# aliabdelkader/FusionTransformer

Hardware: AMD Instinct MI355X
Metric: frames/sec fwd+bwd (SemanticKITTI synth), whole job (higher is better)
Workload: dtype f32

## Files before the change

### fusiontransformer_amd/_lib.py

```python
from __future__ import annotations

import ctypes as C
import os

import torch

_HERE = os.path.dirname(os.path.abspath(__file__))
LIB_PATH = os.path.join(_HERE, "csrc", "libftx.so")

_i32, _i64, _f32, _vp, _sz = C.c_int32, C.c_int64, C.c_float, C.c_void_p, C.c_size_t

SIGNATURES = {
    "ftx_version": (C.c_int, []),
    "ftx_last_error": (C.c_char_p, []),
    "ftx_stream_scratch_bytes": (_sz, []),
    "ftx_stream_scratch_attach": (C.c_int, [_vp, _vp, _sz]),
    "ftx_stream_scratch_reset": (C.c_int, [_vp]),
    "ftx_stream_scratch_release": (C.c_int, [_vp]),
    "ftx_hash": (C.c_int, [_vp, _i64, _vp, _vp]),
    "ftx_hash_kernel": (C.c_int, [_vp, _i64, _vp, _i32, _vp, _vp]),
    "ftx_floor_coords": (C.c_int, [_vp, _i64, _i32, _vp, _vp]),
    "ftx_hashtable_capacity": (_i64, [_i64]),
    "ftx_hashtable_build": (C.c_int, [_vp, _i64, _vp, _vp, _i64, _vp]),
    "ftx_hashtable_query": (C.c_int, [_vp, _i64, _vp, _vp, _i64, _vp, _vp]),
# ... 18 lines not shown
    "ftx_devoxelize_fwd": (C.c_int, [_vp, _vp, _vp, _i64, _i32, _i64, _vp, _vp]),
    "ftx_devoxelize_bwd": (C.c_int, [_vp, _vp, _vp, _i64, _i32, _i64, _vp, _vp]),
    "ftx_segment_workspace_bytes": (_sz, [_i64, _i64]),
    "ftx_segment_build": (C.c_int, [_vp, _i64, _i64, _vp, _vp, _vp, _sz, _vp]),
    "ftx_voxelize_fwd_sorted": (C.c_int, [_vp, _vp, _vp, _i64, _i32, _i64, _vp, _vp]),
    "ftx_devoxelize_bwd_sorted": (C.c_int, [_vp, _vp, _vp, _vp, _i64, _i32, _i64, _vp, _vp]),
    "ftx_segment_sum": (C.c_int, [_vp, _vp, _vp, _i64, _i32, _i64, _vp, _vp]),
    "ftx_lift_cells": (C.c_int, [_vp, _vp, _i64, _i32, _i32, _i32, _i32, _i32, _vp, _vp]),
    "ftx_lift_gather_fwd": (C.c_int, [_vp, _vp, _vp, _i64, _i32, _i32, _i32, _i32, _i32, _i32, _vp, _vp]),
    "ftx_lift_gather_bwd": (C.c_int, [_vp, _vp, _vp, _i64, _i32, _i32, _i32, _i32, _i32, _i32, _vp, _vp]),
    "ftx_resample_nearest_fwd": (C.c_int, [_vp, _i32, _i32, _i32, _i32, _i32, _i32, _vp, _vp]),
    "ftx_resample_nearest_bwd": (C.c_int, [_vp, _i32, _i32, _i32, _i32, _i32, _i32, _vp, _vp]),
    "ftx_sample_down_workspace_bytes": (_sz, []),
    "ftx_sample_down_fwd": (C.c_int, [_vp, _i32, _i32, _i32, _i32, _i32, _vp, _vp, _vp, _vp, _vp, _vp, _f32, _f32, _i32, _vp, _vp, _vp, _sz, _vp]),
    "ftx_sample_down_bwd": (C.c_int, [_vp, _vp, _i32, _i32, _i32, _i32, _i32, _vp, _vp, _vp, _vp, _vp, _vp, _vp, _vp, _vp, _sz, _vp]),
    "ftx_affine_sample_fwd": (C.c_int, [_vp, _vp, _i32, _i32, _i32, _i32, _vp, _i32, _i32, _vp, _vp]),
    "ftx_affine_theta_workspace_bytes": (_sz, [_i32]),
    "ftx_affine_sample_bwd_theta": (C.c_int, [_vp, _vp, _i32, _i32, _i32, _i32, _vp, _vp, _i32, _i32, _vp, _vp, _sz, _vp]),
    "ftx_affine_lift_fwd": (C.c_int, [_vp, _vp, _i32, _i32, _i32, _i32, _vp, _vp, _vp, _i64, _i32, _i32, _vp, _vp]),
    "ftx_affine_lift_cells": (C.c_int, [_vp, _vp, _vp, _i64, _i32, _i32, _i32, _i32, _i32, _vp, _vp]),
    "ftx_affine_lift_bwd": (C.c_int, [_vp, _vp, _i32, _i32, _i32, _i32, _vp, _vp, _vp, _vp, _i64, _i32, _i32, _vp, _vp, _vp, _vp, _vp, _sz, _vp]),
    "ftx_loc_conv_pool_relu_fwd_workspace_bytes": (_sz, [_i32, _i32, _i32, _i32]),
    "ftx_loc_conv_pool_relu_fwd": (C.c_int, [_vp, _vp, _i32, _i32, _i32, _i32, _vp, _vp, _i32, _i32, _vp, _vp, _vp, _vp, _sz, _vp]),
    "ftx_loc_conv_pool_relu_bwd_weight_workspace_bytes": (_sz, [_i32, _i32, _i32, _i32, _i32, _i32]),
    "ftx_loc_conv_pool_relu_bwd_weight": (C.c_int, [_vp, _vp, _i32, _i32, _i32, _i32, _vp, _vp, _vp, _i32, _i32, _vp, _vp, _vp, _sz, _vp]),
    "ftx_loc_conv_pool_relu_bwd_data": (C.c_int, [_vp, _vp, _vp, _vp, _i32, _i32, _i32, _i32, _i32, _i32, _vp, _vp, _vp]),
    "ftx_spconv_pairs_gemm": (C.c_int, [_vp, _i64, _vp, _vp, _i32, _vp, _i64, _i32, _i32, _i32, _vp, _vp]),
    "ftx_spconv_pairs_gemm_scatter": (C.c_int, [_vp, _i64, _vp, _vp, _vp, _i32, _vp, _i64, _i32, _i32, _i32, _vp, _i64, _vp]),
    "ftx_spconv_ostat_supported": (_i32, [_i32, _i32, _i32, _i32]),
    "ftx_spconv_ostat_blocks": (_i32, [_i64]),
    "ftx_spconv_ostat": (C.c_int, [_vp, _i64, _vp, _i64, _vp, _i32, _i32, _i32, _i32, _i32, _vp, _vp, _i32, _vp]),
    "ftx_rows_gemm": (C.c_int, [_vp, _i64, _vp, _i32, _vp, _i32, _i32, _vp, _vp]),
    "ftx_spconv_gemm_block_cols": (_i32, [_i32, _i64, _i32]),
    "ftx_spconv_reduce": (C.c_int, [_vp, _vp, _i64, _i32, _i32, _vp, _vp]),
    "ftx_spconv_reduce_bn_eval": (C.c_int, [_vp, _vp, _i64, _i32, _i32, _vp, _vp, _vp, _vp, _vp, _f32, _i32, _vp, _vp]),
    "ftx_spconv_reduce_stats_blocks": (_i32, [_i64, _i32]),
    "ftx_spconv_reduce_stats": (C.c_int, [_vp, _vp, _i64, _i32, _i32, _vp, _vp, _i32, _vp]),
    "ftx_bn_train_fwd_totals": (C.c_int, [_vp, _vp, _vp, _vp, _vp, _vp, _f32, _f32, _i64, _i32, _i32, _vp, _vp, _vp, _vp, _vp]),
    "ftx_spconv_pairs_wgrad_workspace_bytes": (_sz, [_i64, _i32, _i32, _i32]),
    "ftx_spconv_pairs_wgrad": (C.c_int, [_vp, _i64, _vp, _vp, _i64, _vp, _vp, _i64, _i32, _i32, _i32, _vp, _vp, _sz, _vp]),
    "ftx_spconv_wgrad_resident_blocks": (_i32, [_i32, _i32]),
    "ftx_spconv_wgrad_table_blocks": (_i32, [_i32, _i32, _i32, _i32]),
    "ftx_spconv_pairs_gemm_bf16": (C.c_int, [_vp, _i64, _vp, _vp, _i32, _vp, _i64, _i32, _i32, _i32, _vp, _vp]),
    "ftx_spconv_pairs_gemm_scatter_bf16": (C.c_int, [_vp, _i64, _vp, _vp, _vp, _i32, _vp, _i64, _i32, _i32, _i32, _vp, _i64, _vp]),
    "ftx_rows_gemm_bf16": (C.c_int, [_vp, _i64, _vp, _i32, _vp, _i32, _i32, _vp, _vp]),
    "ftx_spconv_pairs_wgrad_bf16_workspace_bytes": (_sz, [_i64, _i32, _i32, _i32]),
    "ftx_spconv_pairs_wgrad_bf16": (C.c_int, [_vp, _i64, _vp, _vp, _i64, _vp, _vp, _i64, _i32, _i32, _i32, _vp, _vp, _sz, _vp]),
    "ftx_spconv_gemm_bf16_block_cols": (_i32, [_i32, _i64, _i32]),
    "ftx_spconv_wgrad_bf16_table_blocks": (_i32, [_i32, _i32, _i32, _i32]),
    "ftx_bn_workspace_bytes": (_sz, [_i64, _i32]),
    "ftx_bn_train_fwd": (C.c_int, [_vp, _vp, _vp, _vp, _vp, _vp, _f32, _f32, _i64, _i32, _i32, _vp, _vp, _vp, _vp, _sz, _vp]),
    "ftx_bn_eval_fwd": (C.c_int, [_vp, _vp, _vp, _vp, _vp, _vp, _f32, _i64, _i32, _i32, _vp, _vp]),
    "ftx_adam_chunk_elements": (_i32, []),
    "ftx_adam_tensor_bytes": (_i32, []),
    "ftx_adam_step": (C.c_int, [_vp, _vp, _vp, _i32, C.c_double, C.c_double, _f32, _f32, _vp]),
    "ftx_add_layernorm_fwd": (C.c_int, [_vp, _vp, _vp, _vp, _vp, _f32, _i64, _i32, _vp, _vp, _vp, _vp, _vp]),
    "ftx_layernorm_bwd_workspace_bytes": (_sz, [_i64, _i32]),
    "ftx_add_layernorm_bwd": (C.c_int, [_vp, _vp, _vp, _vp, _vp, _vp, _i64, _i32, _i32, _vp, _vp, _vp, _sz, _vp]),
    "ftx_colsum_workspace_bytes": (_sz, [_i64, _i32]),
    "ftx_colsum": (C.c_int, [_vp, _i64, _i32, _vp, _vp, _sz, _vp]),
    "ftx_attn_fwd": (C.c_int, [_vp, _i32, _i32, _i32, _i32, _f32, _vp, _vp, _vp]),
    "ftx_attn_bwd_workspace_bytes": (_sz, [_i32, _i32, _i32]),
    "ftx_attn_bwd": (C.c_int, [_vp, _vp, _vp, _vp, _i32, _i32, _i32, _i32, _f32, _vp, _vp, _sz, _vp]),
    "ftx_attn_fwd_tiled": (C.c_int, [_vp, _i32, _i32, _i32, _i32, _f32, _vp, _vp, _i32, _i32, _vp]),
    "ftx_attn_bwd_tiled": (C.c_int, [_vp, _vp, _vp, _vp, _i32, _i32, _i32, _i32, _f32, _vp, _vp, _sz, _i32, _i32, _vp]),
    "ftx_attn_fwd_bf16": (C.c_int, [_vp, _i32, _i32, _i32, _i32, _f32, _vp, _vp, _i32, _i32, _vp]),
# ... 105 lines not shown
```

### fusiontransformer_amd/csrc/ftx_spconv.hip

```cpp
#include <cstring>
#include <cstdlib>
#include "ftx_bn_eval_op.h"
#include "ftx_spconv_common.h"
#include <rocprim/device/device_scan.hpp>
#include <rocprim/iterator/transform_iterator.hpp>

using namespace ftx;

struct IsValid {
  __host__ __device__ int32_t operator()(int32_t v) const { return v >= 0 ? 1 : 0; }
};

extern "C" size_t ftx_kernel_map_count_workspace_bytes(int64_t n_out, int32_t k) {
  if (n_out <= 0 || k <= 0) return 256;
  size_t bytes = 0;
  const int32_t *in = nullptr;
  int32_t *out = nullptr;
  auto it = rocprim::make_transform_iterator(in, IsValid());
  if (rocprim::exclusive_scan(nullptr, bytes, it, out, 0, (size_t)(n_out * k), rocprim::plus<int32_t>()) != hipSuccess) return 0;
  return bytes + 256;
}

__global__ void koff_kernel(const int32_t *__restrict__ nbr, const int32_t *__restrict__ scan, int64_t n_out, int k, int32_t *__restrict__ koff) {
  int t = blockIdx.x * blockDim.x + threadIdx.x;
// ... 162 lines not shown
        int nn = e >> 3, k4 = (e & 7) * 4;
        *(float4 *)&Bs[nn * BS_STRIDE + k4] = rb[q];
      }
    }
  };

  load_chunk(0);
  for (int c0 = 0; c0 < ca; c0 += kPairBK) {
    store_chunk();
    __syncthreads();
    if (c0 + kPairBK < ca) load_chunk(c0 + kPairBK);
    const float *arow_p = &As[(wave * 32 + l31) * AS_STRIDE + 4 * half];
    const float *brow_p = &Bs[l31 * BS_STRIDE + 4 * half];
    float af[2][4], bf[2][NT][4];
    auto load_frag = [&](int buf, int t) {
      float4 a = *(const float4 *)(arow_p + 8 * t);
      af[buf][0] = a.x; af[buf][1] = a.y; af[buf][2] = a.z; af[buf][3] = a.w;
#pragma unroll
      for (int j = 0; j < NT; ++j) {
        float4 b = *(const float4 *)(brow_p + j * 32 * BS_STRIDE + 8 * t);
        bf[buf][j][0] = b.x; bf[buf][j][1] = b.y; bf[buf][j][2] = b.z; bf[buf][j][3] = b.w;
      }
    };
    load_frag(0, 0);
#pragma unroll
    for (int t = 0; t < kPairBK / 8; ++t) {
      if (t + 1 < kPairBK / 8) load_frag((t + 1) & 1, t + 1);
#pragma unroll
      for (int s = 0; s < 4; ++s)
#pragma unroll
        for (int j = 0; j < NT; ++j) acc[j] = __builtin_amdgcn_mfma_f32_32x32x2f32(bf[t & 1][j][s], af[t & 1][s], acc[j], 0, 0, 0);
    }
    __syncthreads();
  }
  pair_gemm_epilogue<NT>(acc, p0, cnt, n0, gather, rows_a, scatter, rows_out, bias, co, tmp);
}

#include "ftx_lastblock.h"


template <int KVOL>
__device__ __forceinline__ float4 reduce_row(const float *__restrict__ tmp, const int32_t *__restrict__ pos, int64_t n, int co, int kvol,
                                             int64_t r, int j) {
  float4 acc = make_float4(0.f, 0.f, 0.f, 0.f);
  if (KVOL > 0) {
    int32_t p[KVOL > 0 ? KVOL : 1];
#pragma unroll
    for (int k = 0; k < KVOL; ++k) p[k] = pos[(int64_t)k * n + r];
#pragma unroll
    for (int k = 0; k < KVOL; ++k) {
      if (p[k] >= 0) {
        float4 v = *(const float4 *)&tmp[(int64_t)p[k] * co + j];
        acc.x += v.x; acc.y += v.y; acc.z += v.z; acc.w += v.w;
      }
    }
  } else {
    for (int k = 0; k < kvol; ++k) {
      int32_t q = pos[(int64_t)k * n + r];
      if (q >= 0) {
        float4 v = *(const float4 *)&tmp[(int64_t)q * co + j];
        acc.x += v.x; acc.y += v.y; acc.z += v.z; acc.w += v.w;
      }
    }
  }
  return acc;
}
// ... 275 lines not shown
    float *dst = single ? dW + (int64_t)k * mat : part + (int64_t)blockIdx.x * mat;
    const int ab = m0 + wm * 32 * MI + MI * l31, gb = n0 + wn * 32 * NI;
#pragma unroll
    for (int i = 0; i < MI; ++i) {
      const int row = ab + i;
      if (row < ca) {
#pragma unroll
        for (int q = 0; q < 4; ++q) {
          float v[4 * NI];
#pragma unroll
          for (int e = 0; e < 4; ++e)
#pragma unroll
            for (int j = 0; j < NI; ++j) v[e * NI + j] = acc[i][j][4 * q + e];
          const int col = gb + NI * (8 * q + 4 * half);
#pragma unroll
          for (int t = 0; t < NI; ++t)
            if (col + 4 * t < cg) *(float4 *)&dst[(int64_t)row * cg + col + 4 * t] = make_float4(v[4 * t], v[4 * t + 1], v[4 * t + 2], v[4 * t + 3]);
        }
      }
    }
  }
}

struct SpconvF32 {
  static constexpr const char *pairs_name = "ftx_spconv_pairs_gemm", *scatter_name = "ftx_spconv_pairs_gemm_scatter", *rows_name = "ftx_rows_gemm",
                              *wgrad_name = "ftx_spconv_pairs_wgrad";
  static constexpr int wgrad_blocks[4][4] = {{8, 4, 3, 3}, {5, 3, 2, 2}, {4, 2, 1, 2}, {3, 2, 2, 2}};
  static constexpr int wgrad_step = 2 * WG_BR;
  template <int NT>
  static void gemm(dim3 grid, hipStream_t st, const PairsGemmArgs &a) {
    pairs_gemm_kernel<NT><<<grid, 256, 0, st>>>(a.A, a.rows_a, a.gather, a.W, a.w_transposed, a.koff, a.ca, a.co, a.kvol, a.out, a.bias, a.n_dense,
                                                a.scatter, a.rows_out);
  }
  template <int MI, int NI, int WMG, int WNG>
  static void wgrad(dim3 grid, hipStream_t st, const PairsWgradArgs &a) {
    pairs_wgrad_kernel<MI, NI, WMG, WNG><<<grid, 256, 0, st>>>(a.A, a.rows_a, a.idx_a, a.G, a.rows_g, a.idx_g, a.koff, a.ca, a.cg, a.kvol, a.tile_len,
                                                               a.part, a.dW, a.n_dense);
  }
};

extern "C" int32_t ftx_spconv_gemm_block_cols(int32_t co, int64_t n_pairs, int32_t kvol) { return spconv_gemm_block_cols(co, n_pairs, kvol); }

extern "C" int ftx_spconv_pairs_gemm(const float *A, int64_t rows_a, const int32_t *gather, const float *W, int32_t w_transposed,
                                     const int32_t *koff, int64_t n_pairs, int32_t ca, int32_t co, int32_t kvol, float *tmp, void *stream) {
  return spconv_pairs_entry<SpconvF32>(false, A, rows_a, gather, nullptr, W, w_transposed, koff, n_pairs, ca, co, kvol, tmp, 0, stream);
}

extern "C" int ftx_spconv_pairs_gemm_scatter(const float *A, int64_t rows_a, const int32_t *gather, const int32_t *scatter, const float *W,
                                             int32_t w_transposed, const int32_t *koff, int64_t n_pairs, int32_t ca, int32_t co, int32_t kvol,
                                             float *out, int64_t rows_out, void *stream) {
  return spconv_pairs_entry<SpconvF32>(true, A, rows_a, gather, scatter, W, w_transposed, koff, n_pairs, ca, co, kvol, out, rows_out, stream);
}

extern "C" int ftx_rows_gemm(const float *A, int64_t n, const float *W, int32_t w_transposed, const float *bias, int32_t ca, int32_t co,
                             float *out, void *stream) {
  return spconv_rows_entry<SpconvF32>(A, n, W, w_transposed, bias, ca, co, out, stream);
}

extern "C" int32_t ftx_spconv_wgrad_table_blocks(int32_t mi, int32_t wmg, int32_t ni, int32_t wng) {
  return spconv_wgrad_table_blocks<SpconvF32>(mi, wmg, ni, wng);
}
extern "C" int32_t ftx_spconv_wgrad_resident_blocks(int32_t ca, int32_t cg) { return spconv_wgrad_occ<SpconvF32>(spconv_wgrad_config(ca, cg)); }

extern "C" size_t ftx_spconv_pairs_wgrad_workspace_bytes(int64_t n_pairs, int32_t ca, int32_t cg, int32_t kvol) {
  return spconv_wgrad_workspace_bytes<SpconvF32>(n_pairs, ca, cg, kvol);
}

extern "C" int ftx_spconv_pairs_wgrad(const float *A, int64_t rows_a, const int32_t *idx_a, const float *G, int64_t rows_g, const int32_t *idx_g,
                                      const int32_t *koff, int64_t n_pairs, int32_t ca, int32_t cg, int32_t kvol, float *dW, void *workspace,
                                      size_t workspace_bytes, void *stream) {
  return spconv_wgrad_entry<SpconvF32>(A, rows_a, idx_a, G, rows_g, idx_g, koff, n_pairs, ca, cg, kvol, dW, workspace, workspace_bytes, stream);
}
```

### fusiontransformer_amd/csrc/ftx_spconv_common.h

```cpp
#pragma once
#include "ftx_common.h"
#include "ftx_mfma.h"

namespace ftx {

constexpr int kPairTile = 128;
constexpr int kPairBK = 32;
constexpr int kPairAPasses = 4;
constexpr int kWgradRound = 1024;
constexpr int kWgradCUs = 256;

template <bool RANGE>
__device__ __forceinline__ void pair_tile_scan(const int32_t *__restrict__ koff, int kvol, int tile, int n_dense, int *s_tile) {
  const int tid = threadIdx.x, b = blockIdx.x;
  if (tid >= 64) return;
  int c = 0;
  if (tid < kvol) c = koff ? koff[tid + 1] - koff[tid] : n_dense;
  int nt = (c + tile - 1) / tile;
  int incl = nt;
#pragma unroll
  for (int off = 1; off < 64; off <<= 1) {
    int v = __shfl_up(incl, off, 64);
    if (tid >= off) incl += v;
  }
  int excl = incl - nt;
  bool mine = (tid < kvol) && b >= excl && b < incl;
  unsigned long long m = __ballot(mine);
  if (mine) {
    int t = b - excl;
    int left = c - t * tile;
    int first = (koff ? koff[tid] : 0) + t * tile;
    s_tile[0] = tid;
    s_tile[1] = first;
    s_tile[2] = (RANGE ? first : 0) + (left > tile ? tile : left);
    if (RANGE) s_tile[3] = nt;
  }
  if (m == 0ull && tid == 0) s_tile[0] = -1;
}

__device__ __forceinline__ void gemm_tile_scan(const int32_t *__restrict__ koff, int kvol, int64_t n_dense, bool dense, int *s_tile) {
  if (!dense) {
    __builtin_assume(koff != nullptr);
    return pair_tile_scan<false>(koff, kvol, kPairTile, 0, s_tile);
  }
  if (threadIdx.x == 0) {
    int64_t left = n_dense - (int64_t)blockIdx.x * kPairTile;
    s_tile[0] = left > 0 ? 0 : -1;
    s_tile[1] = blockIdx.x * kPairTile;
    s_tile[2] = left > kPairTile ? kPairTile : (int)left;
  }
}

__device__ __forceinline__ void pair_gather_rows(const int32_t *__restrict__ gather, int p0, int cnt, int64_t rows_a, int32_t (&src)[kPairAPasses]) {
  const int arow = threadIdx.x >> 3;
#pragma unroll
  for (int p = 0; p < kPairAPasses; ++p) {
    int r = p * 32 + arow;
    int32_t s = 0;
    if (r < cnt) s = gather ? gather[p0 + r] : p0 + r;
    if (s < 0 || s >= rows_a) s = 0;
    src[p] = s;
  }
}

template <int NT>
__device__ __forceinline__ void pair_gemm_epilogue(const f32x16 (&acc)[NT], int p0, int cnt, int n0, const int32_t *__restrict__ gather, int64_t rows_a,
                                          const int32_t *__restrict__ scatter, int64_t rows_out, const float *__restrict__ bias, int co,
                                          float *__restrict__ out) {
  const int wave = threadIdx.x >> 6, lane = threadIdx.x & 63;
  const int half = lane >> 5, l31 = lane & 31;
  const bool nfull = n0 + 32 * NT <= co;
  const int row = wave * 32 + l31;
  int64_t drow = row < cnt ? p0 + row : -1;
  bool zero = false;
  if (gather != nullptr && drow >= 0) {
    const int32_t sidx = gather[drow];
    zero = sidx < 0 || sidx >= rows_a;
  }
  if (scatter != nullptr && drow >= 0) {
    drow = scatter[drow];
    if (drow >= rows_out) drow = -1;
  }
// ... 134 lines not shown
  else if (big_tiles <= 32)
    wgrad_reduce_kernel<4><<<rgrid(64), 256, 0, st>>>(part, koff, kvol, tile_len, n_dense, mat, dW);
  else
    wgrad_reduce_kernel<16><<<rgrid(16), 256, 0, st>>>(part, koff, kvol, tile_len, n_dense, mat, dW);
}

struct PairsGemmArgs {
  const float *A;
  int64_t rows_a;
  const int32_t *gather;
  const float *W;
  int w_transposed;
  const int32_t *koff;
  int ca, co, kvol;
  float *out;
  const float *bias;
  int64_t n_dense;
  const int32_t *scatter;
  int64_t rows_out;
};

inline int spconv_gemm_nt(int co, int64_t row_tiles) {
  int nt = co >= 128 ? 4 : (co + 31) / 32;
  if (co > 128 && co % 96 == 0 && co % 128 != 0) nt = 3;
  if (nt == 4 && row_tiles * ceil_div(co, 128) <= 400) nt = 2;
  return nt;
}

inline int32_t spconv_gemm_block_cols(int32_t co, int64_t n_pairs, int32_t kvol) {
  if (co < 4 || co % 4 != 0 || n_pairs < 0 || kvol < 0) return -1;
  return 32 * spconv_gemm_nt(co, ceil_div(n_pairs, kPairTile) + kvol);
}

template <class F>
void spconv_launch_gemm(int64_t row_tiles, hipStream_t st, const PairsGemmArgs &a) {
  const int nt = spconv_gemm_nt(a.co, row_tiles);
  const dim3 grid((unsigned)row_tiles, (unsigned)ceil_div(a.co, 32 * nt));
  switch (nt) {
    case 1: F::template gemm<1>(grid, st, a); break;
    case 2: F::template gemm<2>(grid, st, a); break;
    case 3: F::template gemm<3>(grid, st, a); break;
    default: F::template gemm<4>(grid, st, a); break;
  }
}

template <class F>
int spconv_pairs_entry(bool scattered, const float *A, int64_t rows_a, const int32_t *gather, const int32_t *scatter, const float *W,
                       int32_t w_transposed, const int32_t *koff, int64_t n_pairs, int32_t ca, int32_t co, int32_t kvol, float *out, int64_t rows_out,
                       void *stream) {
  const char *me = scattered ? F::scatter_name : F::pairs_name;
  FTX_REQUIRE(n_pairs >= 0 && rows_a >= 0 && rows_out >= 0 && kvol >= 1 && kvol <= 64, "%s: bad size", me);
  FTX_REQUIRE(ca >= 4 && ca % 4 == 0 && co >= 4 && co % 4 == 0, "%s: channels must be multiples of 4 (ca=%d co=%d)", me, ca, co);
  if (n_pairs == 0) return FTX_OK;
  FTX_REQUIRE(A && gather && (scatter || !scattered) && W && koff && out && rows_a >= 1, "%s: null pointer or empty operand", me);
  const PairsGemmArgs a = {A, rows_a, gather, W, w_transposed, koff, ca, co, kvol, out, nullptr, 0, scatter, rows_out};
  spconv_launch_gemm<F>(ceil_div(n_pairs, kPairTile) + kvol, (hipStream_t)stream, a);
  return check_launch(me);
}

template <class F>
int spconv_rows_entry(const float *A, int64_t n, const float *W, int32_t w_transposed, const float *bias, int32_t ca, int32_t co, float *out,
                      void *stream) {
  const char *me = F::rows_name;
  FTX_REQUIRE(n >= 0, "%s: n < 0", me);
  FTX_REQUIRE(ca >= 4 && ca % 4 == 0 && co >= 4 && co % 4 == 0, "%s: channels must be multiples of 4 (ca=%d co=%d)", me, ca, co);
  if (n == 0) return FTX_OK;
  FTX_REQUIRE(A && W && out, "%s: null pointer", me);
  const PairsGemmArgs a = {A, n, nullptr, W, w_transposed, nullptr, ca, co, 1, out, bias, n, nullptr, 0};
  spconv_launch_gemm<F>(ceil_div(n, kPairTile), (hipStream_t)stream, a);
  return check_launch(me);
}

struct PairsWgradArgs {
  const float *A;
  int64_t rows_a;
  const int32_t *idx_a;
  const float *G;
  int64_t rows_g;
  const int32_t *idx_g, *koff;
  int ca, cg, kvol, tile_len;
  float *part, *dW;
  int n_dense;
};

struct WgradCfg { int mi, wmg, ni, wng; };
inline WgradCfg spconv_wgrad_config(int ca, int cg) {
  WgradCfg c;
  if (ca <= 32) { c.mi = 1; c.wmg = 1; }
  else if (ca <= 64) { c.mi = 2; c.wmg = 1; }
  else if (ca % 96 == 0 && ca % 128 != 0) { c.mi = 3; c.wmg = 1; }
  else { c.mi = 2; c.wmg = 2; }
  if (cg <= 32) { c.ni = 1; c.wng = 1; }
  else if (cg <= 64) { c.ni = 2; c.wng = 1; }
  else if (cg % 96 == 0 && cg % 128 != 0) { c.ni = 3; c.wng = 1; }
  else { c.ni = 2; c.wng = 2; }
  if (c.mi == 3 && c.ni == 3) { c.mi = 2; c.wmg = 2; }
  return c;
}

template <class F>
int spconv_wgrad_occ(const WgradCfg &c) {
  auto side = [](int i, int w) { return w == 2 ? 3 : i - 1; };
// ... 84 lines not shown
```

### include/ftx.h

```cpp
#ifndef FTX_H
#define FTX_H

#include <stddef.h>
#include <stdint.h>

#ifdef __cplusplus
extern "C" {
#endif

#define FTX_OK 0
#define FTX_EINVAL -1
#define FTX_ELAUNCH -2
#define FTX_EWORKSPACE -3

int ftx_version(void);
const char *ftx_last_error(void);

size_t ftx_stream_scratch_bytes(void);
int ftx_stream_scratch_attach(void *stream, void *buffer, size_t bytes);
int ftx_stream_scratch_reset(void *stream);
int ftx_stream_scratch_release(void *stream);


int ftx_hash(const int32_t *coords, int64_t n, int64_t *out, void *stream);
// ... 52 lines not shown
int ftx_lift_cells(const int64_t *img_idx, const int32_t *point_batch, int64_t n, int32_t b, int32_t gh, int32_t gw, int32_t H, int32_t W, int32_t *cells, void *stream);

int ftx_resample_nearest_fwd(const float *in, int32_t b, int32_t c, int32_t ih, int32_t iw, int32_t oh, int32_t ow, float *out, void *stream);
int ftx_resample_nearest_bwd(const float *grad_out, int32_t b, int32_t c, int32_t ih, int32_t iw, int32_t oh, int32_t ow, float *grad_in, void *stream);

size_t ftx_sample_down_workspace_bytes(void);
int ftx_sample_down_fwd(const float *img, int32_t b, int32_t h, int32_t w, int32_t oh, int32_t ow, const float *conv_w, const float *conv_b, const float *gamma, const float *beta, float *running_mean, float *running_var, float momentum, float eps, int32_t training, float *out, double *saved, void *workspace, size_t workspace_bytes, void *stream);
int ftx_sample_down_bwd(const float *img, const float *grad_out, int32_t b, int32_t h, int32_t w, int32_t oh, int32_t ow, const float *conv_w, const float *conv_b, const float *gamma, const double *saved, float *grad_conv_w, float *grad_conv_b, float *grad_gamma, float *grad_beta, void *workspace, size_t workspace_bytes, void *stream);

int ftx_affine_sample_fwd(const float *src, const int64_t *src_strides, int32_t b, int32_t c, int32_t ih, int32_t iw, const float *theta, int32_t oh, int32_t ow, float *out, void *stream);
size_t ftx_affine_theta_workspace_bytes(int32_t b);
int ftx_affine_sample_bwd_theta(const float *src, const int64_t *src_strides, int32_t b, int32_t c, int32_t ih, int32_t iw, const float *theta, const float *grad_out, int32_t oh, int32_t ow, float *grad_theta, void *workspace, size_t workspace_bytes, void *stream);
int ftx_affine_lift_fwd(const float *src, const int64_t *src_strides, int32_t b, int32_t c, int32_t ih, int32_t iw, const float *theta, const int64_t *img_idx, const int32_t *point_batch, int64_t n, int32_t H, int32_t W, float *out, void *stream);
int ftx_affine_lift_cells(const float *theta, const int64_t *img_idx, const int32_t *point_batch, int64_t n, int32_t b, int32_t ih, int32_t iw, int32_t H, int32_t W, int32_t *cells, void *stream);
int ftx_affine_lift_bwd(const float *src, const int64_t *src_strides, int32_t b, int32_t c, int32_t ih, int32_t iw, const float *theta, const int64_t *img_idx, const int32_t *point_batch, const float *grad_out, int64_t n, int32_t H, int32_t W, const int32_t *order, const int32_t *seg_off, float *grad_src, float *grad_theta, void *workspace, size_t workspace_bytes, void *stream);

size_t ftx_loc_conv_pool_relu_fwd_workspace_bytes(int32_t b, int32_t co, int32_t ph, int32_t pw);
int ftx_loc_conv_pool_relu_fwd(const float *x, const int64_t *x_strides, int32_t b, int32_t c, int32_t ih, int32_t iw, const float *w, const float *bias, int32_t k, int32_t co, float *out, int8_t *sel, float *mean, void *workspace, size_t workspace_bytes, void *stream);
size_t ftx_loc_conv_pool_relu_bwd_weight_workspace_bytes(int32_t b, int32_t c, int32_t ih, int32_t iw, int32_t k, int32_t co);
int ftx_loc_conv_pool_relu_bwd_weight(const float *x, const int64_t *x_strides, int32_t b, int32_t c, int32_t ih, int32_t iw, const int8_t *sel, const float *grad, const int64_t *grad_strides, int32_t k, int32_t co, float *grad_w, float *grad_bias, void *workspace, size_t workspace_bytes, void *stream);
int ftx_loc_conv_pool_relu_bwd_data(const float *w, const int8_t *sel, const float *grad, const int64_t *grad_strides, int32_t b, int32_t c, int32_t ih, int32_t iw, int32_t k, int32_t co, float *grad_x, const int64_t *grad_x_strides, void *stream);


int ftx_spconv_pairs_gemm(const float *A, int64_t rows_a, const int32_t *gather, const float *W, int32_t w_transposed, const int32_t *koff, int64_t n_pairs, int32_t ca, int32_t co, int32_t kvol, float *tmp, void *stream);

int ftx_spconv_pairs_gemm_scatter(const float *A, int64_t rows_a, const int32_t *gather, const int32_t *scatter, const float *W, int32_t w_transposed, const int32_t *koff, int64_t n_pairs, int32_t ca, int32_t co, int32_t kvol, float *out, int64_t rows_out, void *stream);

int32_t ftx_spconv_ostat_supported(int32_t ca, int32_t co, int32_t kvol, int32_t w_transposed);
int32_t ftx_spconv_ostat_blocks(int64_t n_out);
int ftx_spconv_ostat(const float *A, int64_t rows_a, const int32_t *nbr, int64_t n_out, const float *W, int32_t w_transposed, int32_t flip, int32_t ca, int32_t co, int32_t kvol, float *out, double *part, int32_t nb, void *stream);

int ftx_rows_gemm(const float *A, int64_t n, const float *W, int32_t w_transposed, const float *bias, int32_t ca, int32_t co, float *out, void *stream);
int32_t ftx_spconv_gemm_block_cols(int32_t co, int64_t n_pairs, int32_t kvol);

int ftx_spconv_reduce(const float *tmp, const int32_t *pos, int64_t n, int32_t co, int32_t kvol, float *out, void *stream);

int ftx_spconv_reduce_bn_eval(const float *tmp, const int32_t *pos, int64_t n, int32_t co, int32_t kvol, const float *residual, const float *gamma, const float *beta, const float *running_mean, const float *running_var, float eps, int32_t relu, float *out, void *stream);

int32_t ftx_spconv_reduce_stats_blocks(int64_t n, int32_t co);
int ftx_spconv_reduce_stats(const float *tmp, const int32_t *pos, int64_t n, int32_t co, int32_t kvol, float *out, double *part, int32_t nb, void *stream);

size_t ftx_spconv_pairs_wgrad_workspace_bytes(int64_t n_pairs, int32_t ca, int32_t cg, int32_t kvol);
int ftx_spconv_pairs_wgrad(const float *A, int64_t rows_a, const int32_t *idx_a, const float *G, int64_t rows_g, const int32_t *idx_g, const int32_t *koff, int64_t n_pairs, int32_t ca, int32_t cg, int32_t kvol, float *dW, void *workspace, size_t workspace_bytes, void *stream);
int32_t ftx_spconv_wgrad_resident_blocks(int32_t ca, int32_t cg);
int32_t ftx_spconv_wgrad_table_blocks(int32_t mi, int32_t wmg, int32_t ni, int32_t wng);

int ftx_spconv_pairs_gemm_bf16(const float *A, int64_t rows_a, const int32_t *gather, const float *W, int32_t w_transposed, const int32_t *koff, int64_t n_pairs, int32_t ca, int32_t co, int32_t kvol, float *tmp, void *stream);
int ftx_spconv_pairs_gemm_scatter_bf16(const float *A, int64_t rows_a, const int32_t *gather, const int32_t *scatter, const float *W, int32_t w_transposed, const int32_t *koff, int64_t n_pairs, int32_t ca, int32_t co, int32_t kvol, float *out, int64_t rows_out, void *stream);
int ftx_rows_gemm_bf16(const float *A, int64_t n, const float *W, int32_t w_transposed, const float *bias, int32_t ca, int32_t co, float *out, void *stream);
size_t ftx_spconv_pairs_wgrad_bf16_workspace_bytes(int64_t n_pairs, int32_t ca, int32_t cg, int32_t kvol);
int ftx_spconv_pairs_wgrad_bf16(const float *A, int64_t rows_a, const int32_t *idx_a, const float *G, int64_t rows_g, const int32_t *idx_g, const int32_t *koff, int64_t n_pairs, int32_t ca, int32_t cg, int32_t kvol, float *dW, void *workspace, size_t workspace_bytes, void *stream);
int32_t ftx_spconv_gemm_bf16_block_cols(int32_t co, int64_t n_pairs, int32_t kvol);
int32_t ftx_spconv_wgrad_bf16_table_blocks(int32_t mi, int32_t wmg, int32_t ni, int32_t wng);


size_t ftx_bn_workspace_bytes(int64_t n, int32_t c);
int ftx_bn_train_fwd(const float *x, const float *residual, const float *gamma, const float *beta, float *running_mean, float *running_var, float momentum, float eps, int64_t n, int32_t c, int32_t relu, float *y, float *save_mean, float *save_invstd, void *workspace, size_t workspace_bytes, void *stream);
int ftx_bn_train_fwd_totals(const float *x, const float *residual, const float *gamma, const float *beta, float *running_mean, float *running_var, float momentum, float eps, int64_t n, int32_t c, int32_t relu, float *y, float *save_mean, float *save_invstd, const double *totals, void *stream);

int ftx_bn_eval_fwd(const float *x, const float *residual, const float *gamma, const float *beta, const float *running_mean, const float *running_var, float eps, int64_t n, int32_t c, int32_t relu, float *y, void *stream);
int ftx_bn_train_bwd(const float *grad_y, const float *x, const float *y, const float *gamma, const float *beta, const float *save_mean, const float *save_invstd, int64_t n, int32_t c, int32_t relu, float *grad_x, float *grad_residual, float *grad_gamma, float *grad_beta, void *workspace, size_t workspace_bytes, void *stream);

int32_t ftx_adam_chunk_elements(void);
int32_t ftx_adam_tensor_bytes(void);
int ftx_adam_step(const void *table, const int32_t *chunk_tensor, const int64_t *chunk_offset, int32_t n_chunks, double beta1, double beta2, float eps, float weight_decay, void *stream);

// ... 114 lines not shown
```

Measured before the change: 148.3.

## Add ping-pong 512-thread pair GEMM kernel with staggered weight loading

Adds an fp32 sparse-conv pair GEMM variant that runs two 256-thread groups per block on a 256-row tile. The two groups share a double-buffered weight tile whose loads are staggered by one chunk, so one group's loads overlap the other's MFMA work. An automatic heuristic selects it for large channel counts (ca and co at least 128, co a multiple of 128) when enough blocks exist, and an explicit variant entry point is exposed. The aim is to hide global-load latency and halve weight staging per row, at the cost of more LDS per block, extra template instantiations and a more complex synchronisation scheme.

New measurement: 144.7. 0.976x the previous value.

```diff
diff --git a/fusiontransformer_amd/_lib.py b/fusiontransformer_amd/_lib.py
--- a/fusiontransformer_amd/_lib.py
+++ b/fusiontransformer_amd/_lib.py
@@ -74,6 +74,8 @@
     "ftx_spconv_ostat": (C.c_int, [_vp, _i64, _vp, _i64, _vp, _i32, _i32, _i32, _i32, _i32, _vp, _vp, _i32, _vp]),
     "ftx_rows_gemm": (C.c_int, [_vp, _i64, _vp, _i32, _vp, _i32, _i32, _vp, _vp]),
     "ftx_spconv_gemm_block_cols": (_i32, [_i32, _i64, _i32]),
+    "ftx_spconv_gemm_variant": (C.c_int, [_vp, _i64, _vp, _vp, _vp, _i32, _vp, _vp, _i64, _i32, _i32, _i32, _vp, _i64, _i32, _vp]),
+    "ftx_spconv_gemm_pingpong": (_i32, [_i32, _i32, _i64, _i32]),
     "ftx_spconv_reduce": (C.c_int, [_vp, _vp, _i64, _i32, _i32, _vp, _vp]),
     "ftx_spconv_reduce_bn_eval": (C.c_int, [_vp, _vp, _i64, _i32, _i32, _vp, _vp, _vp, _vp, _vp, _f32, _i32, _vp, _vp]),
     "ftx_spconv_reduce_stats_blocks": (_i32, [_i64, _i32]),
diff --git a/fusiontransformer_amd/csrc/ftx_spconv.hip b/fusiontransformer_amd/csrc/ftx_spconv.hip
--- a/fusiontransformer_amd/csrc/ftx_spconv.hip
+++ b/fusiontransformer_amd/csrc/ftx_spconv.hip
@@ -218,6 +218,155 @@
         for (int j = 0; j < NT; ++j) acc[j] = __builtin_amdgcn_mfma_f32_32x32x2f32(bf[t & 1][j][s], af[t & 1][s], acc[j], 0, 0, 0);
     }
     __syncthreads();
+  }
+  pair_gemm_epilogue<NT>(acc, p0, cnt, n0, gather, rows_a, scatter, rows_out, bias, co, tmp);
+}
+
+template <int NT, bool WT, bool KFULL>
+__global__ __launch_bounds__(512, 4) void pairs_gemm_pp_kernel(const float *__restrict__ A, int64_t rows_a, const int32_t *__restrict__ gather,
+                                                               const float *__restrict__ W, const int32_t *__restrict__ koff,
+                                                               int ca, int co, int kvol, float *__restrict__ tmp, const float *__restrict__ bias,
+                                                               int64_t n_dense, const int32_t *__restrict__ scatter, int64_t rows_out) {
+  constexpr bool w_transposed = WT, kfull = KFULL;
+  constexpr int BN = 32 * NT;
+  constexpr int BS_STRIDE = AS_STRIDE;
+  constexpr int A_PASSES = kPairAPasses;
+
+  __shared__ __attribute__((aligned(16))) float As2[2][kPairTile * AS_STRIDE];
+  __shared__ __attribute__((aligned(16))) float Bs2[2][BN * BS_STRIDE];
+  __shared__ int s_tile[3];
+
+  gemm_tile_scan_pp(koff, kvol, n_dense, gather == nullptr, s_tile);
+  __syncthreads();
+  const int k = __builtin_amdgcn_readfirstlane(s_tile[0]);
+  if (k < 0) return;
+  const int p0 = __builtin_amdgcn_readfirstlane(s_tile[1]), cnt = __builtin_amdgcn_readfirstlane(s_tile[2]);
+
+  const int grp = __builtin_amdgcn_readfirstlane((int)(threadIdx.x >> 8));
+  const int tid = threadIdx.x & 255;
+  const int wave = tid >> 6, lane = tid & 63;
+  const int half = lane >> 5, l31 = lane & 31;
+  const int n0 = blockIdx.y * BN;
+  const int arow = tid >> 3, acol = (tid & 7) * 4;
+  const int gp0 = p0 + grp * kPairTile, gcnt = cnt - grp * kPairTile;
+  const bool live = gcnt > 0;
+  const int nchunk = (ca + kPairBK - 1) / kPairBK;
+  float *As = As2[grp];
+
+  int32_t src[A_PASSES];
+#pragma unroll
+  for (int p = 0; p < A_PASSES; ++p) {
+    int r = p * 32 + arow;
+    int32_t s = 0;
+    if (r < gcnt) s = gather ? gather[gp0 + r] : gp0 + r;
+    if (s < 0 || s >= rows_a) s = 0;
+    src[p] = s;
+  }
+  const float *Wk = W + (int64_t)k * ca * co;
+
+  f32x16 acc[NT];
+#pragma unroll
+  for (int j = 0; j < NT; ++j)
+#pragma unroll
+    for (int g = 0; g < 16; ++g) acc[j][g] = 0.f;
+
+  float4 ra[A_PASSES], rb0, rb1 = make_float4(0.f, 0.f, 0.f, 0.f);
+  auto load_a = [&](int c0) {
+#pragma unroll
+    for (int p = 0; p < A_PASSES; ++p) {
+      float4 v = make_float4(0.f, 0.f, 0.f, 0.f);
+      if (kfull || c0 + acol < ca) v = *(const float4 *)&A[(int64_t)src[p] * ca + c0 + acol];
+      ra[p] = v;
+    }
+  };
+  auto load_w1 = [&](int q, int c0) -> float4 {
+    if (kfull) {
+      if (!w_transposed) {
+        int kk = ((tid >> 6) << 3) + (tid & 7), n4 = n0 + (q * 8 + ((tid >> 3) & 7)) * 4;
+        n4 = n4 + 4 <= co ? n4 : co - 4;
+        return *(const float4 *)&Wk[(int64_t)(c0 + kk) * co + n4];
+      }
+      int e = q * 256 + tid;
+      int nn = n0 + (e >> 3), k4 = (e & 7) * 4;
+      nn = nn < co ? nn : co - 1;
+      return *(const float4 *)&Wk[(int64_t)nn * ca + c0 + k4];
+    }
+    float4 v = make_float4(0.f, 0.f, 0.f, 0.f);
+    if (!w_transposed) {
+      int kk = ((tid >> 6) << 3) + (tid & 7), n4 = (q * 8 + ((tid >> 3) & 7)) * 4;
+      if (c0 + kk < ca && n0 + n4 < co) v = *(const float4 *)&Wk[(int64_t)(c0 + kk) * co + n0 + n4];
+    } else {
+      int e = q * 256 + tid;
+      int nn = e >> 3, k4 = (e & 7) * 4;
+      if (n0 + nn < co && c0 + k4 < ca) v = *(const float4 *)&Wk[(int64_t)(n0 + nn) * ca + c0 + k4];
+    }
+    return v;
+  };
+  const bool two_w = NT % 2 == 0 || grp == 0;
+  auto load_w = [&](int c0) {
+    rb0 = load_w1(grp, c0);
+    if (two_w) rb1 = load_w1(2 + grp, c0);
+  };
+  auto store_a = [&]() {
+#pragma unroll
+    for (int p = 0; p < A_PASSES; ++p) *(float4 *)&As[(p * 32 + arow) * AS_STRIDE + acol] = ra[p];
+  };
+  auto store_w1 = [&](float *Bs, int q, const float4 &v) {
+    if (!w_transposed) {
+      int kk = ((tid >> 6) << 3) + (tid & 7), n4 = (q * 8 + ((tid >> 3) & 7)) * 4;
+      Bs[(n4 + 0) * BS_STRIDE + kk] = v.x;
+      Bs[(n4 + 1) * BS_STRIDE + kk] = v.y;
+      Bs[(n4 + 2) * BS_STRIDE + kk] = v.z;
+      Bs[(n4 + 3) * BS_STRIDE + kk] = v.w;
+    } else {
+      int e = q * 256 + tid;
+      int nn = e >> 3, k4 = (e & 7) * 4;
+      *(float4 *)&Bs[nn * BS_STRIDE + k4] = v;
+    }
+  };
+  auto store_w = [&](float *Bs) {
+    store_w1(Bs, grp, rb0);
+    if (two_w) store_w1(Bs, 2 + grp, rb1);
+  };
+  auto mfma_chunk = [&](const float *Bs) {
+    const float *arow_p = &As[(wave * 32 + l31) * AS_STRIDE + 4 * half];
+    const float *brow_p = &Bs[l31 * BS_STRIDE + 4 * half];
+    float4 a = *(const float4 *)arow_p, b = *(const float4 *)brow_p;
+#pragma unroll
+    for (int t = 0; t < kPairBK / 8; ++t) {
+      float4 an = a;
+      if (t + 1 < kPairBK / 8) an = *(const float4 *)(arow_p + 8 * (t + 1));
+#pragma unroll
+      for (int j = 0; j < NT; ++j) {
+        const int jn = j + 1 < NT ? j + 1 : 0, tn = j + 1 < NT ? t : t + 1;
+        float4 bn = b;
+        if (tn < kPairBK / 8) bn = *(const float4 *)(brow_p + jn * 32 * BS_STRIDE + 8 * tn);
+        acc[j] = __builtin_amdgcn_mfma_f32_32x32x2f32(b.x, a.x, acc[j], 0, 0, 0);
+        acc[j] = __builtin_amdgcn_mfma_f32_32x32x2f32(b.y, a.y, acc[j], 0, 0, 0);
+        acc[j] = __builtin_amdgcn_mfma_f32_32x32x2f32(b.z, a.z, acc[j], 0, 0, 0);
+        acc[j] = __builtin_amdgcn_mfma_f32_32x32x2f32(b.w, a.w, acc[j], 0, 0, 0);
+        b = bn;
+      }
+      a = an;
+    }
+  };
+
+  if (grp == 1) {
+    load_w(0);
+    store_w(Bs2[0]);
+  }
+  if (live) load_a(0);
+  if (grp < nchunk) load_w(grp * kPairBK);
+  if (grp == 1) __syncthreads();
+  for (int c = 0; c < nchunk; ++c) {
+    const int wc = c + grp;
+    if (live) store_a();
+    if (wc < nchunk) store_w(Bs2[wc & 1]);
+    if (live && c + 1 < nchunk) load_a((c + 1) * kPairBK);
+    if (wc + 1 < nchunk) load_w((wc + 1) * kPairBK);
+    __syncthreads();
+    mfma_chunk(Bs2[c & 1]);
+    if (grp == 0 || c + 1 < nchunk) __syncthreads();
   }
   pair_gemm_epilogue<NT>(acc, p0, cnt, n0, gather, rows_a, scatter, rows_out, bias, co, tmp);
 }
@@ -559,6 +708,18 @@
     pairs_gemm_kernel<NT><<<grid, 256, 0, st>>>(a.A, a.rows_a, a.gather, a.W, a.w_transposed, a.koff, a.ca, a.co, a.kvol, a.out, a.bias, a.n_dense,
                                                 a.scatter, a.rows_out);
   }
+  static constexpr bool pingpong = true;
+  template <int NT, bool WT, bool KFULL>
+  static void gemm_pp_form(dim3 grid, hipStream_t st, const PairsGemmArgs &a) {
+    pairs_gemm_pp_kernel<NT, WT, KFULL><<<grid, 512, 0, st>>>(a.A, a.rows_a, a.gather, a.W, a.koff, a.ca, a.co, a.kvol, a.out, a.bias, a.n_dense,
+                                                              a.scatter, a.rows_out);
+  }
+  template <int NT>
+  static void gemm_pp(dim3 grid, hipStream_t st, const PairsGemmArgs &a) {
+    const bool kfull = a.ca % kPairBK == 0;
+    if (a.w_transposed) kfull ? gemm_pp_form<NT, true, true>(grid, st, a) : gemm_pp_form<NT, true, false>(grid, st, a);
+    else kfull ? gemm_pp_form<NT, false, true>(grid, st, a) : gemm_pp_form<NT, false, false>(grid, st, a);
+  }
   template <int MI, int NI, int WMG, int WNG>
   static void wgrad(dim3 grid, hipStream_t st, const PairsWgradArgs &a) {
     pairs_wgrad_kernel<MI, NI, WMG, WNG><<<grid, 256, 0, st>>>(a.A, a.rows_a, a.idx_a, a.G, a.rows_g, a.idx_g, a.koff, a.ca, a.cg, a.kvol, a.tile_len,
@@ -584,6 +745,26 @@
   return spconv_rows_entry<SpconvF32>(A, n, W, w_transposed, bias, ca, co, out, stream);
 }
 
+extern "C" int32_t ftx_spconv_gemm_pingpong(int32_t ca, int32_t co, int64_t n_pairs, int32_t kvol) {
+  if (ca < 4 || co < 4 || n_pairs < 0 || kvol < 0) return 0;
+  return spconv_gemm_pingpong(ca, co, n_pairs, kvol) ? 1 : 0;
+}
+
+extern "C" int ftx_spconv_gemm_variant(const float *A, int64_t rows_a, const int32_t *gather, const int32_t *scatter, const float *W,
+                                       int32_t w_transposed, const float *bias, const int32_t *koff, int64_t n_pairs, int32_t ca, int32_t co,
+                                       int32_t kvol, float *out, int64_t rows_out, int32_t variant, void *stream) {
+  const char *me = "ftx_spconv_gemm_variant";
+  FTX_REQUIRE(variant == kGemmAuto || variant == kGemmFourWave || variant == kGemmPingPong, "%s: variant must be 0 (automatic), 1 (four waves) or 2 (ping-pong), got %d", me, variant);
+  FTX_REQUIRE(variant != kGemmPingPong || (co >= 4 && spconv_gemm_pp_nt(co) != 0), "%s: the ping-pong kernel is built for co > 64 only (co=%d)", me, co);
+  if (gather == nullptr) {
+    FTX_REQUIRE(scatter == nullptr && koff == nullptr && kvol == 1, "%s: dense rows (gather NULL) take no scatter list, no koff and kvol 1", me);
+    return spconv_rows_entry<SpconvF32>(A, n_pairs, W, w_transposed, bias, ca, co, out, stream, variant);
+  }
+  FTX_REQUIRE(bias == nullptr, "%s: a pair list takes no bias", me);
+  return spconv_pairs_entry<SpconvF32>(scatter != nullptr, A, rows_a, gather, scatter, W, w_transposed, koff, n_pairs, ca, co, kvol, out,
+                                       scatter != nullptr ? rows_out : 0, stream, variant);
+}
+
 extern "C" int32_t ftx_spconv_wgrad_table_blocks(int32_t mi, int32_t wmg, int32_t ni, int32_t wng) {
   return spconv_wgrad_table_blocks<SpconvF32>(mi, wmg, ni, wng);
 }
diff --git a/fusiontransformer_amd/csrc/ftx_spconv_common.h b/fusiontransformer_amd/csrc/ftx_spconv_common.h
--- a/fusiontransformer_amd/csrc/ftx_spconv_common.h
+++ b/fusiontransformer_amd/csrc/ftx_spconv_common.h
@@ -5,6 +5,7 @@
 namespace ftx {
 
 constexpr int kPairTile = 128;
+constexpr int kPairTilePP = 256;
 constexpr int kPairBK = 32;
 constexpr int kPairAPasses = 4;
 constexpr int kWgradRound = 1024;
@@ -48,6 +49,19 @@
     s_tile[0] = left > 0 ? 0 : -1;
     s_tile[1] = blockIdx.x * kPairTile;
     s_tile[2] = left > kPairTile ? kPairTile : (int)left;
+  }
+}
+
+__device__ __forceinline__ void gemm_tile_scan_pp(const int32_t *__restrict__ koff, int kvol, int64_t n_dense, bool dense, int *s_tile) {
+  if (!dense) {
+    __builtin_assume(koff != nullptr);
+    return pair_tile_scan<false>(koff, kvol, kPairTilePP, 0, s_tile);
+  }
+  if (threadIdx.x == 0) {
+    int64_t left = n_dense - (int64_t)blockIdx.x * kPairTilePP;
+    s_tile[0] = left > 0 ? 0 : -1;
+    s_tile[1] = blockIdx.x * kPairTilePP;
+    s_tile[2] = left > kPairTilePP ? kPairTilePP : (int)left;
   }
 }
 
@@ -248,8 +262,35 @@
   return 32 * spconv_gemm_nt(co, ceil_div(n_pairs, kPairTile) + kvol);
 }
 
-template <class F>
-void spconv_launch_gemm(int64_t row_tiles, hipStream_t st, const PairsGemmArgs &a) {
+enum { kGemmAuto = 0, kGemmFourWave = 1, kGemmPingPong = 2 };
+template <class F, class = void> struct HasPingPong { static constexpr bool value = false; };
+template <class F> struct HasPingPong<F, decltype((void)F::pingpong)> { static constexpr bool value = F::pingpong; };
+
+inline int spconv_gemm_pp_nt(int co) {
+  const int nt = co >= 128 ? 4 : (co + 31) / 32;
+  if (co > 128 && co % 96 == 0 && co % 128 != 0) return 3;
+  return nt >= 3 ? nt : 0;
+}
+
+inline bool spconv_gemm_pingpong(int ca, int co, int64_t n_pairs, int kvol) {
+  if (kvol < 1 || ca < 128 || co < 128 || co % 128 != 0) return false;
+  const int64_t blocks = (ceil_div(n_pairs, kPairTilePP) + kvol) * (co / 128);
+  return blocks >= 2 * kWgradCUs * 15 / 16;
+}
+
+template <class F>
+void spconv_launch_gemm(int64_t n_rows, int kvol_tiles, int variant, hipStream_t st, const PairsGemmArgs &a) {
+  if constexpr (HasPingPong<F>::value) {
+    if (variant == kGemmAuto) variant = spconv_gemm_pingpong(a.ca, a.co, n_rows, kvol_tiles) ? kGemmPingPong : kGemmFourWave;
+    if (variant == kGemmPingPong) {
+      const int nt = spconv_gemm_pp_nt(a.co);
+      const dim3 grid((unsigned)(ceil_div(n_rows, kPairTilePP) + kvol_tiles), (unsigned)ceil_div(a.co, 32 * nt));
+      if (nt == 3) F::template gemm_pp<3>(grid, st, a);
+      else F::template gemm_pp<4>(grid, st, a);
+      return;
+    }
+  }
+  const int64_t row_tiles = ceil_div(n_rows, kPairTile) + kvol_tiles;
   const int nt = spconv_gemm_nt(a.co, row_tiles);
   const dim3 grid((unsigned)row_tiles, (unsigned)ceil_div(a.co, 32 * nt));
   switch (nt) {
@@ -263,27 +304,27 @@
 template <class F>
 int spconv_pairs_entry(bool scattered, const float *A, int64_t rows_a, const int32_t *gather, const int32_t *scatter, const float *W,
                        int32_t w_transposed, const int32_t *koff, int64_t n_pairs, int32_t ca, int32_t co, int32_t kvol, float *out, int64_t rows_out,
-                       void *stream) {
+                       void *stream, int variant = kGemmAuto) {
   const char *me = scattered ? F::scatter_name : F::pairs_name;
   FTX_REQUIRE(n_pairs >= 0 && rows_a >= 0 && rows_out >= 0 && kvol >= 1 && kvol <= 64, "%s: bad size", me);
   FTX_REQUIRE(ca >= 4 && ca % 4 == 0 && co >= 4 && co % 4 == 0, "%s: channels must be multiples of 4 (ca=%d co=%d)", me, ca, co);
   if (n_pairs == 0) return FTX_OK;
   FTX_REQUIRE(A && gather && (scatter || !scattered) && W && koff && out && rows_a >= 1, "%s: null pointer or empty operand", me);
   const PairsGemmArgs a = {A, rows_a, gather, W, w_transposed, koff, ca, co, kvol, out, nullptr, 0, scatter, rows_out};
-  spconv_launch_gemm<F>(ceil_div(n_pairs, kPairTile) + kvol, (hipStream_t)stream, a);
+  spconv_launch_gemm<F>(n_pairs, kvol, variant, (hipStream_t)stream, a);
   return check_launch(me);
 }
 
 template <class F>
 int spconv_rows_entry(const float *A, int64_t n, const float *W, int32_t w_transposed, const float *bias, int32_t ca, int32_t co, float *out,
-                      void *stream) {
+                      void *stream, int variant = kGemmAuto) {
   const char *me = F::rows_name;
   FTX_REQUIRE(n >= 0, "%s: n < 0", me);
   FTX_REQUIRE(ca >= 4 && ca % 4 == 0 && co >= 4 && co % 4 == 0, "%s: channels must be multiples of 4 (ca=%d co=%d)", me, ca, co);
   if (n == 0) return FTX_OK;
   FTX_REQUIRE(A && W && out, "%s: null pointer", me);
   const PairsGemmArgs a = {A, n, nullptr, W, w_transposed, nullptr, ca, co, 1, out, bias, n, nullptr, 0};
-  spconv_launch_gemm<F>(ceil_div(n, kPairTile), (hipStream_t)stream, a);
+  spconv_launch_gemm<F>(n, 0, variant, (hipStream_t)stream, a);
   return check_launch(me);
 }
 
diff --git a/include/ftx.h b/include/ftx.h
--- a/include/ftx.h
+++ b/include/ftx.h
@@ -108,6 +108,8 @@
 
 int ftx_rows_gemm(const float *A, int64_t n, const float *W, int32_t w_transposed, const float *bias, int32_t ca, int32_t co, float *out, void *stream);
 int32_t ftx_spconv_gemm_block_cols(int32_t co, int64_t n_pairs, int32_t kvol);
+int ftx_spconv_gemm_variant(const float *A, int64_t rows_a, const int32_t *gather, const int32_t *scatter, const float *W, int32_t w_transposed, const float *bias, const int32_t *koff, int64_t n_pairs, int32_t ca, int32_t co, int32_t kvol, float *out, int64_t rows_out, int32_t variant, void *stream);
+int32_t ftx_spconv_gemm_pingpong(int32_t ca, int32_t co, int64_t n_pairs, int32_t kvol);
 
 int ftx_spconv_reduce(const float *tmp, const int32_t *pos, int64_t n, int32_t co, int32_t kvol, float *out, void *stream);
 
```
